# rajan-dubey8/camouflage-multimodal

Hardware: AMD Instinct MI355X
Metric: images/sec fwd+bwd (fusion model train step: fwd + loss + bwd + clip + AdamW) (higher is better)
Workload: dtype bf16; 1 GPU; BASELINE configs[1] on the path that exists (SURVEY 8d): cross-attention fusion model, packed variable-Nr minibatch (Nr ~ real 303..530 histogram, mean 483), Nk=13 real KG rows, train mode dropout 0.3, random-init weights; batch_per_gpu=16, global_batch=16, rg_dim=128, hidden_dim=256, num_heads=8, parallelism=dp1, precision=bf16 MFMA operands, fp32 accumulate/optimizer

## Files before the change

camouflage_multimodal_amd/csrc/fused_rows.h:

```cpp
#pragma once
#include "common.h"

typedef unsigned short us16;

struct ShadowJob { us16* dst; int N, K, transposed, nsrc; const float* src[4]; int rows[4]; int ld[4]; int chunk_begin; int lo; };
#define SHADOW_MAXJ 24
#define SHADOW_MAXZ 24
struct ShadowBatch { ShadowJob j[SHADOW_MAXJ]; int n; void* zero_ptr[SHADOW_MAXZ]; size_t zero_bytes[SHADOW_MAXZ]; int nzero; };
int launch_weight_shadows(ShadowBatch& sb, hipStream_t stream);

struct FrontStream {
  const float* X; int M;
  const us16* W0; const float* b0;
  const us16* W1; const float* bq; const float* bkv;
  us16* X16;
  us16* R16; us16* Q16; us16* KV16;
  int tile_begin;
};
#define FUSED_FRONT_MAXZ 4
#define FUSED_FRONT_MAXX 20
#define FUSED_BWD1_MAXZ 16
struct FrontArgs {
  FrontStream s[2]; float qscale; int save; unsigned long long* stamps; int exp;
  void* zero_ptr[FUSED_FRONT_MAXZ]; unsigned zero_bytes[FUSED_FRONT_MAXZ]; int nzero;
// ... 2 lines not shown
};
int launch_fused_front(FrontArgs& a, int variant, hipStream_t stream);

struct BackStream {
  const us16* Wo; const float* bo; const us16* W1; const float* b1; const float* ln_g; const float* ln_b;
  const us16* R16;
  us16* O16; us16* Y16; us16* XH16; float* rstd; uint32_t* mask;
  float* Ymean; float* Hmean;
  uint32_t site_ffn;
};
struct BackArgs {
  BackStream s[2];
  const us16* Q16; const us16* KV16;
  const us16* Q2_16; const us16* KV2_16;
  const int* off; const int* tile_off; const float* inv_nr;
  const int4* tile_desc;
  float* lse2;
  int lead_tiles;
  float* part; int* tickets; int max_splits;
  int B, Nk, rg_tiles_max, rows_rg;
  DropCfg drop; int save; int exp;
  unsigned long long* stamps;
  int save_lse2;
};
int launch_fused_back(BackArgs& a, int variant, int lead_mode, hipStream_t stream);

struct Bwd1Stream {
  const us16* W1T; const us16* WoT;
  const uint32_t* mask; const us16* XH16; const float* rstd; const float* ln_g;
  const float* dHm; int ld_dHm;
  const float* dcomb; int ld_dcomb;
  us16* dH16; us16* dU16;
  float* dgamma; float* dbeta;
};
struct TailWgProd { const float* dy; const float* x; float* dW; float* db; int ld_dy, ld_x, rows, cols; int tile_begin; };
#define TAIL_WG_MAXP 8
struct TailWgArgs { TailWgProd p[TAIL_WG_MAXP]; int n, B, tiles; };
struct Bwd1Args {
  Bwd1Stream s[2];
  const us16* Q16; const us16* KV16;
  us16* dQKV16; float* dKV;
  const us16* O2_16; us16* dO2_16; float* delta2;
  const int* off; const int* tile_off; const float* inv_nr; const int4* tile_desc;
  const int* row_sample;
  int B, Nk, rg_tiles_max, rows_rg; float qscale; DropCfg drop; unsigned long long* stamps;
  int exp;
// ... 44 lines not shown
```

camouflage_multimodal_amd/csrc/fused_rows.hip:

```cpp
#include "fused_rows.h"
#include "shadow_inl.h"
#include "gemm.h"
#include "mfma_inl.h"

namespace {

template <int NT, int KS, bool W_IS_A, int DEPTH, bool USE_ROT = true>
struct Stage {
  static constexpr int TOTAL = NT * KS;
  static constexpr int D = DEPTH < TOTAL ? DEPTH : TOTAL;
  static_assert(!USE_ROT || (KS & (KS - 1)) == 0, "rotated k order: power-of-two k steps");
  u32x4 buf[D];
  const u32x4* wp; int rot;
  __device__ __forceinline__ int keff(int ks) const { return USE_ROT ? ((ks + rot) & (KS - 1)) : ks; }
  __device__ __forceinline__ const u32x4* wptr(int i) const { return wp + 64 * (keff(i / NT) * NT + (i % NT)); }
  __device__ __forceinline__ void prefetch(const u32x4* __restrict__ wp_, int rot_) {
    wp = wp_; rot = rot_;
#pragma unroll
    for (int i = 0; i < D; ++i) buf[i] = *wptr(i);
  }
  __device__ __forceinline__ void run(const char* act, f32x16 (&acc)[NT]) {
    run_f([&](int ks) { return *reinterpret_cast<const bf16x8*>(act + 32 * ks); }, acc);
  }
  template <class F>
  __device__ __forceinline__ void run_f(F&& frag, f32x16 (&acc)[NT]) {
    bf16x8 x = frag(keff(0)), xn = x;
#pragma unroll
    for (int i = 0; i < TOTAL; ++i) {
      const int ks = i / NT, t = i % NT;
      const bf16x8 wf = as_frag(buf[i % D]);
      if (i + D < TOTAL) buf[i % D] = *wptr(i + D);
      if (t == 0) {
        x = xn;
        if (ks + 1 < KS) xn = frag(keff(ks + 1));
      }
      if constexpr (W_IS_A) acc[t] = __builtin_amdgcn_mfma_f32_32x32x16_bf16(wf, x, acc[t], 0, 0, 0);
      else                  acc[t] = __builtin_amdgcn_mfma_f32_32x32x16_bf16(x, wf, acc[t], 0, 0, 0);
      __builtin_amdgcn_sched_barrier(0);
    }
  }
};

__device__ __forceinline__ void stamp(unsigned long long* stamps, int k) {
  if (stamps && threadIdx.x == 0) stamps[(size_t)blockIdx.x * 8 + k] = __builtin_amdgcn_s_memrealtime();
}

template <int LOG2C>
__device__ __forceinline__ void copy_out(const char* lds, int pitch, int col_byte0, us16* dst, int ld, size_t row0, int nrows) {
  for (int c = threadIdx.x; c < (32 << LOG2C); c += 256) {
    const int r = c >> LOG2C, k = c & ((1 << LOG2C) - 1);
    if (r < nrows)
      store16_wt(reinterpret_cast<char*>(dst + (row0 + r) * (size_t)ld) + 16 * k, *reinterpret_cast<const u32x4*>(lds + r * pitch + col_byte0 + 16 * k));
  }
}
// ... 125 lines not shown
    for (int s = 0; s < 2; ++s) {
      const bf16x8 kf = *reinterpret_cast<const bf16x8*>(Ks + (l31 & 15) * PK + 2 * (32 * head + 16 * s + 8 * h));
      S = __builtin_amdgcn_mfma_f32_32x32x16_bf16(kf, qf[hd][s], S, 0, 0, 0);
    }
    float e[8];
    rg_softmax(S, h, Nk, e);
    const uint32_t ibase = ((uint32_t)(row0 + l31) * 8u + (uint32_t)head) * (uint32_t)Nk;
    if (dodrop) {
#pragma unroll
      for (int i = 0; i < 8; ++i) e[i] *= drop_mult(a.drop, SITE_ATTN_RG2KG, ibase + (uint32_t)acc_row(i, h));
    }
    const bf16x8 pf = as_frag(u32x4{pack2(e[0], e[1]), pack2(e[2], e[3]), pack2(e[4], e[5]), pack2(e[6], e[7])});
    const char* vp = Vs + (4 * h + q4) * PV + 2 * (32 * head + 16 * g1 + 4 * p4);
    const bf16x8 vf = join(lds_tr16(vp), lds_tr16(vp + 8 * PV));
    const f32x16 O = __builtin_amdgcn_mfma_f32_32x32x16_bf16(vf, pf, zero16(), 0, 0, 0);
#pragma unroll
    for (int g = 0; g < 4; ++g)
      *reinterpret_cast<u32x2*>(bufO + l31 * PR + 2 * (32 * head + 8 * g + 4 * h)) =
          u32x2{pack2(O[4 * g], O[4 * g + 1]), pack2(O[4 * g + 2], O[4 * g + 3])};
  }
}

constexpr int SPLIT_ROWS = 64;
constexpr int PART_FLOATS = 16 + 16 + 16 * 32;
static_assert(PART_FLOATS == FUSED_PART_FLOATS, "fused_rows.h");
__device__ __forceinline__ void attn_kg_split(const BackArgs& a, char* smem, int b, int sp, int w, int lane) {
  const int l31 = lane & 31, h = lane >> 5, Nk = a.Nk;
  const int rb = a.off[b], nr = a.off[b + 1] - rb, r0 = SPLIT_ROWS * sp;
  char* Vt = smem + w * (32 * PVC);
  const us16* qrow = a.Q2_16 + ((size_t)b * Nk + min(l31, Nk - 1)) * 256 + 64 * w + 8 * h;
  const us16* kbase = a.KV2_16 + (size_t)rb * 512 + 64 * w + 8 * h;
  const us16* vbase = a.KV2_16 + (size_t)rb * 512 + 256 + 64 * w;
  bf16x8 qf[2][2];
  u32x4 kf[2][2][2], vv[2][4];
#pragma unroll
  for (int hd = 0; hd < 2; ++hd)
#pragma unroll
    for (int s = 0; s < 2; ++s) qf[hd][s] = as_frag(*reinterpret_cast<const u32x4*>(qrow + 32 * hd + 16 * s));
#pragma unroll
  for (int c = 0; c < 2; ++c) {
    const us16* p = kbase + (size_t)min(r0 + 32 * c + l31, nr - 1) * 512;
#pragma unroll
    for (int hd = 0; hd < 2; ++hd)
#pragma unroll
      for (int s = 0; s < 2; ++s) kf[c][hd][s] = *reinterpret_cast<const u32x4*>(p + 32 * hd + 16 * s);
  }
// ... 50 lines not shown
  L[0] += __shfl_xor(L[0], 32, 64);
  L[1] += __shfl_xor(L[1], 32, 64);
  stamp(a.stamps, 2);
#pragma unroll
  for (int hd = 0; hd < 2; ++hd) {
    float* part = a.part + (((size_t)a.tile_off[b] + 2 * sp) * 8 + 2 * w + hd) * PART_FLOATS;
    if (lane < 16) {
      __hip_atomic_store(part + lane, mx[hd], __ATOMIC_RELAXED, __HIP_MEMORY_SCOPE_AGENT);
      __hip_atomic_store(part + 16 + lane, L[hd], __ATOMIC_RELAXED, __HIP_MEMORY_SCOPE_AGENT);
    }
    float* zt = reinterpret_cast<float*>(Vt);
#pragma unroll
    for (int i = 0; i < 8; ++i) zt[acc_row(i, h) * 32 + l31] = Z[hd][i];
#pragma unroll
    for (int r = 0; r < 2; ++r) {
      const int idx = lane + 64 * r;
      const f32x4 v = *reinterpret_cast<const f32x4*>(zt + 4 * idx);
      float* dst = part + 32 + 4 * idx;
      asm volatile("global_store_dwordx4 %0, %1, off sc1\n\ts_nop 1" ::"v"(dst), "v"(v) : "memory");
    }
  }
}

__device__ __forceinline__ void attn_kg_combine(const BackArgs& a, char* smem, char* bufO, int b, int nsplit) {
  const int tid = threadIdx.x, Nk = a.Nk;
  float* sc = reinterpret_cast<float*>(smem);
  float* invL = sc + nsplit * 128;
  const float* part = a.part + (size_t)a.tile_off[b] * 8 * PART_FLOATS;
  constexpr size_t SS = (size_t)2 * 8 * PART_FLOATS;
  f32x4 zv[4][4];
  auto load_z = [&](int s0) {
#pragma unroll
    for (int k = 0; k < 4; ++k) {
      const float* z = part + (size_t)min(s0 + k, nsplit - 1) * SS + 32;
#pragma unroll
      for (int it = 0; it < 4; ++it) {
        const int idx = tid + 256 * it;
        zv[k][it] = *reinterpret_cast<const f32x4*>(z + (size_t)(idx >> 7) * PART_FLOATS + 4 * (idx & 127));
      }
    }
  };
  load_z(0);
  if (tid < 128) {
    const int hd = tid >> 4, j = tid & 15;
    const float* p0 = part + (size_t)hd * PART_FLOATS + j;
    float M = -INFINITY, L = 0.f;
    if (nsplit <= 16) {
// ... 3 lines not shown
#pragma unroll
      for (int k = 0; k < 16; ++k) M = fmaxf(M, mv[k]);
#pragma unroll
      for (int k = 0; k < 16; ++k)
        if (k < nsplit) { const float e = __expf(mv[k] - M); sc[k * 128 + tid] = e; L = fmaf(lv[k], e, L); }
    } else {
      for (int s0 = 0; s0 < nsplit; s0 += 8) {
        float mv[8];
#pragma unroll
        for (int k = 0; k < 8; ++k) mv[k] = p0[(size_t)min(s0 + k, nsplit - 1) * SS];
#pragma unroll
        for (int k = 0; k < 8; ++k) M = fmaxf(M, mv[k]);
      }
      for (int s0 = 0; s0 < nsplit; s0 += 8) {
        float mv[8], lv[8];
#pragma unroll
        for (int k = 0; k < 8; ++k) { const size_t o = (size_t)min(s0 + k, nsplit - 1) * SS; mv[k] = p0[o]; lv[k] = p0[o + 16]; }
#pragma unroll
        for (int k = 0; k < 8; ++k)
          if (s0 + k < nsplit) { const float e = __expf(mv[k] - M); sc[(s0 + k) * 128 + tid] = e; L = fmaf(lv[k], e, L); }
      }
    }
    invL[tid] = 1.0f / L;
    if ((a.save | a.save_lse2) && a.lse2 && j < Nk) { float* o = a.lse2 + (((size_t)b * 8 + hd) * 16 + j) * 2; o[0] = M; o[1] = L; }
  }
  __syncthreads();
  f32x4 acc[4];
#pragma unroll
  for (int it = 0; it < 4; ++it) acc[it] = f32x4{0.f, 0.f, 0.f, 0.f};
  for (int s0 = 0; s0 < nsplit; s0 += 4) {
    if (s0 > 0) load_z(s0);
#pragma unroll
    for (int k = 0; k < 4; ++k)
      if (s0 + k < nsplit) {
#pragma unroll
        for (int it = 0; it < 4; ++it) acc[it] += zv[k][it] * sc[(s0 + k) * 128 + ((tid + 256 * it) >> 3)];
      }
  }
#pragma unroll
  for (int it = 0; it < 4; ++it) {
    const int idx = tid + 256 * it, hd = idx >> 7, j = (idx >> 3) & 15, f4 = idx & 7;
    if (j < Nk) {
      const float il = invL[hd * 16 + j];
      *reinterpret_cast<u32x2*>(bufO + j * PR + 2 * (32 * hd + 4 * f4)) =
          u32x2{pack2(acc[it][0] * il, acc[it][1] * il), pack2(acc[it][2] * il, acc[it][3] * il)};
    }
  }
}

template <int DEPTH, bool ROT, int OCC>
__global__ __launch_bounds__(256, OCC) void back_kernel(const BackArgs a) {
  extern __shared__ __attribute__((aligned(16))) char smem[];
  const int tid = threadIdx.x, lane = tid & 63, l31 = lane & 31, h = lane >> 5;
  const int w = __builtin_amdgcn_readfirstlane(tid >> 6);
  const int nkg = a.B * a.max_splits;
  const int vid = (int)blockIdx.x < a.lead_tiles ? nkg + (int)blockIdx.x : ((int)blockIdx.x < a.lead_tiles + nkg ? (int)blockIdx.x - a.lead_tiles : (int)blockIdx.x);
  const bool kg = vid < nkg;
  int rot = ROT ? (int)(blockIdx.x >> 3) : 0;
  using L = BackL<OCC>;
  char* bufO = smem + L::O; char* bufY = smem + L::Y;
  float* red = reinterpret_cast<float*>(smem + L::RED);
  float* tile32 = reinterpret_cast<float*>(smem);
  int b; size_t rowg0; int nrows; float inv_n;
  stamp(a.stamps, 0);
  const BackStream& S = a.s[kg ? 1 : 0];
  Stage<2, 16, true, DEPTH> sto;
  Stage<4, 16, false, DEPTH> stf;
  if (!kg) sto.prefetch(reinterpret_cast<const u32x4*>(S.Wo) + (size_t)w * (16 * 2 * 64) + lane, rot);
  if (kg) {
    b = vid / a.max_splits;
    const int sp = vid - b * a.max_splits;
    if (ROT) rot = b;
    const int nsplit = (a.off[b + 1] - a.off[b] + SPLIT_ROWS - 1) / SPLIT_ROWS;
    if (sp >= nsplit) return;
    attn_kg_split(a, smem, b, sp, w, lane);
    stamp(a.stamps, 4);
    asm volatile("s_waitcnt vmcnt(0)" ::: "memory");
    __syncthreads();
    int* flag = reinterpret_cast<int*>(red);
    if (tid == 0) flag[0] = __hip_atomic_fetch_add(a.tickets + b, 1, __ATOMIC_RELAXED, __HIP_MEMORY_SCOPE_AGENT);
    __syncthreads();
    stamp(a.stamps, 5);
    if (flag[0] != nsplit - 1) return;
    if (tid == 0) {
      __builtin_amdgcn_fence(__ATOMIC_ACQUIRE, "agent");
      asm volatile("s_waitcnt vmcnt(0)" ::: "memory");
    }
    for (int c = tid; c < 32 * PR / 16; c += 256) reinterpret_cast<u32x4*>(bufO)[c] = u32x4{0u, 0u, 0u, 0u};
    __syncthreads();
    sto.prefetch(reinterpret_cast<const u32x4*>(S.Wo) + (size_t)w * (16 * 2 * 64) + lane, rot);
    attn_kg_combine(a, smem, bufO, b, nsplit);
    stamp(a.stamps, 6);
    rowg0 = (size_t)b * a.Nk; nrows = a.Nk; inv_n = 1.0f / (float)a.Nk;
  } else {
    const int4 td = a.tile_desc[vid - nkg];
    if (td.x < 0) return;
    b = td.x; rowg0 = td.y; nrows = td.z; inv_n = __int_as_float(td.w);
    attn_rg_tile(a, smem, bufO, b, rowg0, nrows, w, lane);
  }
  __syncthreads();
  stamp(a.stamps, 1);

  const size_t rrow = rowg0 + min(l31, nrows - 1);
  float u[32];
  float rstd_keep = 0.f;
  {
    f32x16 acc[2] = {zero16(), zero16()};
    sto.run(bufO + l31 * PR + 16 * h, acc);
    stf.prefetch(reinterpret_cast<const u32x4*>(S.W1) + (size_t)w * (16 * 4 * 64) + lane, rot);
    float part = 0.f;
#pragma unroll
    for (int t = 0; t < 2; ++t)
#pragma unroll
      for (int g = 0; g < 4; ++g) {
        const int c0 = 64 * w + 32 * t + 8 * g + 4 * h;
        const float4 bv = *reinterpret_cast<const float4*>(S.bo + c0);
        const u32x2 rv = *reinterpret_cast<const u32x2*>(S.R16 + rrow * 256 + c0);
        float* o = u + 16 * t + 4 * g;
        o[0] = acc[t][4 * g] + bv.x + bf_lo(rv.x); o[1] = acc[t][4 * g + 1] + bv.y + bf_hi(rv.x);
        o[2] = acc[t][4 * g + 2] + bv.z + bf_lo(rv.y); o[3] = acc[t][4 * g + 3] + bv.w + bf_hi(rv.y);
        part += (o[0] + o[1]) + (o[2] + o[3]);
      }
    auto row_total = [&](float p, int slot) {
      p += __shfl_xor(p, 32, 64);
      if (h == 0) red[slot * 128 + w * 32 + l31] = p;
      __syncthreads();
      return (red[slot * 128 + l31] + red[slot * 128 + 32 + l31]) + (red[slot * 128 + 64 + l31] + red[slot * 128 + 96 + l31]);
    };
    const float mean = row_total(part, 0) * (1.0f / 256.0f);
    float sq = 0.f;
#pragma unroll
    for (int i = 0; i < 32; ++i) { u[i] -= mean; sq = fmaf(u[i], u[i], sq); }
// ... 12 lines not shown
        const float4 y = make_float4(x0 * gm.x + bt.x, x1 * gm.y + bt.y, x2 * gm.z + bt.z, x3 * gm.w + bt.w);
        *reinterpret_cast<u32x2*>(bufY + l31 * PR + 2 * c0) = u32x2{pack2(y.x, y.y), pack2(y.z, y.w)};
        if constexpr (OCC == 3) {
          ys[4 * g] = rok ? y.x : 0.f; ys[4 * g + 1] = rok ? y.y : 0.f; ys[4 * g + 2] = rok ? y.z : 0.f; ys[4 * g + 3] = rok ? y.w : 0.f;
          if (a.save) *reinterpret_cast<u32x2*>(smem + L::XH + l31 * PR + 2 * c0) = u32x2{pack2(x0, x1), pack2(x2, x3)};
        } else {
          *reinterpret_cast<float4*>(tile32 + l31 * PT + c0) = y;
          o[0] = x0; o[1] = x1; o[2] = x2; o[3] = x3;
        }
      }
      if constexpr (OCC == 2) continue;
#pragma unroll
      for (int st = 0; st < 4; ++st) {
        const int n = 8 >> st, m = 16 >> st;
        const bool up = (l31 & m) != 0;
#pragma unroll
        for (int i = 0; i < n; ++i) {
          const float send = up ? ys[i] : ys[i + n];
          const float keep = up ? ys[i + n] : ys[i];
          ys[i] = keep + __shfl_xor(send, m, 64);
        }
      }
      const float tot = ys[0] + __shfl_xor(ys[0], 1, 64);
      if ((l31 & 1) == 0) {
        const int i16 = (l31 >> 1) & 15;
        atomicAdd(S.Ymean + (size_t)b * 256 + 64 * w + 32 * t + 8 * (i16 >> 2) + 4 * h + (i16 & 3), tot * inv_n);
      }
    }
  }
  __syncthreads();
  stamp(a.stamps, 2);
  if constexpr (OCC == 2) {
    float sum = 0.f;
    for (int r = 0; r < nrows; ++r) sum += tile32[r * PT + tid];
    atomicAdd(S.Ymean + (size_t)b * 256 + tid, sum * inv_n);
  }

  {
    f32x16 acc[4] = {zero16(), zero16(), zero16(), zero16()};
    stf.run(bufY + l31 * PR + 16 * h, acc);
    const bool dodrop = a.drop.p > 0.f;
#pragma unroll
    for (int t = 0; t < 4; ++t) {
      const int f = 128 * w + 32 * t + l31;
      const float bias = S.b1[f];
      float colsum = 0.f;
      uint32_t wlo = 0u, whi = 0u;
#pragma unroll
      for (int i = 0; i < 16; ++i) {
        if (8 * (i >> 2) >= nrows) continue;
        const int row = acc_row(i, h);
        float v = fmaxf(acc[t][i] + bias, 0.f);
        if (dodrop) v *= drop_mult(a.drop, S.site_ffn, (uint32_t)(rowg0 + row) * 512u + (uint32_t)f);
        if (row >= nrows) v = 0.f;
        colsum += v;
        if (a.save) {
          const unsigned long long bal = __ballot(v > 0.f);
          SET_LANE(wlo, (uint32_t)bal, i); SET_LANE(whi, (uint32_t)(bal >> 32), i);
        }
      }
      colsum += __shfl_xor(colsum, 32, 64);
      if (h == 0) atomicAdd(S.Hmean + (size_t)b * 512 + f, colsum * inv_n);
      if (a.save && lane < 16) {
        const int ra = acc_row(lane, 0);
        if (ra < nrows) S.mask[(rowg0 + ra) * 16 + 4 * w + t] = wlo;
        if (ra + 4 < nrows) S.mask[(rowg0 + ra + 4) * 16 + 4 * w + t] = whi;
      }
    }
  }
  if (a.save) {
    char* bufXH = smem + L::XH;
    if (w == 0 && h == 0 && l31 < nrows) S.rstd[rowg0 + l31] = rstd_keep;
    __syncthreads();
    if constexpr (OCC == 2) {
#pragma unroll
      for (int t = 0; t < 2; ++t)
#pragma unroll
        for (int g = 0; g < 4; ++g) {
          const float* o = u + 16 * t + 4 * g;
          *reinterpret_cast<u32x2*>(bufXH + l31 * PR + 2 * (64 * w + 32 * t + 8 * g + 4 * h)) = u32x2{pack2(o[0], o[1]), pack2(o[2], o[3])};
        }
      __syncthreads();
    }
    copy_out<5>(bufXH, PR, 0, S.XH16, 256, rowg0, nrows);
    copy_out<5>(bufO, PR, 0, S.O16, 256, rowg0, nrows);
    copy_out<5>(bufY, PR, 0, S.Y16, 256, rowg0, nrows);
  }
  stamp(a.stamps, 3);
}


constexpr int W_GTAB = 0, W_BUFDU = 1024, W_KS = W_BUFDU + 32 * PR, W_VS = W_KS + 16 * PK, W_BUFDO = W_VS + 16 * PK,
              W_IMGS = W_BUFDO + 32 * PR, W_RED = W_IMGS + 16384, W_LDS = W_RED + 1024;
// ... 763 lines not shown
    total += (S.M + 31) / 32;
  }
  if (a.nzero < 0 || a.nzero > FUSED_FRONT_MAXZ) return (int)hipErrorInvalidValue;
  for (int i = 0; i < a.nzero; ++i)
    if (!a.zero_ptr[i] || !al16(a.zero_ptr[i]) || (a.zero_bytes[i] & 15)) return (int)hipErrorInvalidValue;
  const int prof = gemm_prof_open(stream, 2.0 * ((double)a.s[0].M + a.s[1].M) * (128.0 * 256.0 + 256.0 * 768.0), PROF_FRONT);
  if (variant == 0)      launch_lds<front_kernel<12, false>>(dim3(total), dim3(256), F_LDS, stream, a);
  else if (variant != 2) launch_lds<front_kernel<12, true>>(dim3(total), dim3(256), F_LDS, stream, a);
  else                   launch_lds<front_kernel<16, true>>(dim3(total), dim3(256), F_LDS, stream, a);
  gemm_prof_close(prof, stream);
  return (int)hipGetLastError();
}

int launch_fused_back(BackArgs& a, int variant, int lead_mode, hipStream_t stream) {
  if (a.B < 1 || a.Nk < 1 || a.Nk > 16 || a.rg_tiles_max < 1 || !a.Q16 || !a.KV16 || !a.Q2_16 || !a.KV2_16 || !a.off || !a.tile_off || !a.tile_desc || !a.inv_nr ||
      !a.part || !a.tickets || a.max_splits < 1 || a.max_splits > FUSED_MAX_SPLITS)
    return (int)hipErrorInvalidValue;
  for (int i = 0; i < 2; ++i) {
    const BackStream& S = a.s[i];
    if (!S.Wo || !S.bo || !S.W1 || !S.b1 || !S.ln_g || !S.ln_b || !S.R16 || !S.Ymean || !S.Hmean) return (int)hipErrorInvalidValue;
    if (a.save && (!S.O16 || !S.Y16 || !S.XH16 || !S.rstd || !S.mask)) return (int)hipErrorInvalidValue;
    if (!al16(S.bo) || !al16(S.ln_g) || !al16(S.ln_b) || !al16(S.Wo) || !al16(S.W1) || !al16(S.R16)) return (int)hipErrorInvalidValue;
  }
  const dim3 grid(a.B * a.max_splits + a.rg_tiles_max);
  a.lead_tiles = (lead_mode != 0 && a.rows_rg / 32 >= 256 && (int)grid.x > 512) ? 256 : 0;
  const double rows = (double)a.rows_rg + (double)a.B * a.Nk;
  const int prof = gemm_prof_open(stream, 2.0 * rows * (256.0 * 256.0 + 256.0 * 512.0) + 8.0 * (double)a.rows_rg * a.Nk * 256.0, PROF_BACK);
  if (variant == 0)        launch_lds<back_kernel<12, false, 2>>(grid, dim3(256), BackL<2>::LDS, stream, a);
  else if (variant != 2) {
    if (grid.x <= 512u)    launch_lds<back_kernel<12, true, 2>>(grid, dim3(256), BackL<2>::LDS, stream, a);
    else                   launch_lds<back_kernel<12, true, 3>>(grid, dim3(256), BackL<3>::LDS, stream, a);
  } else                   launch_lds<back_kernel<16, true, 2>>(grid, dim3(256), BackL<2>::LDS, stream, a);
  gemm_prof_close(prof, stream);
  return (int)hipGetLastError();
}

size_t fused_bwd1_lds() { return W_LDS; }

int launch_fused_bwd1(Bwd1Args& a, int variant, hipStream_t stream, int kg_only) {
  if (a.B < 1 || a.Nk < 1 || a.Nk > 16 || a.rg_tiles_max < 1 || !a.Q16 || !a.KV16 || !a.dQKV16 || !a.dKV || !a.O2_16 || !a.dO2_16 || !a.delta2 ||
      !a.off || !a.tile_off || !a.tile_desc || !a.inv_nr || !a.row_sample)
    return (int)hipErrorInvalidValue;
  for (int i = 0; i < 2; ++i) {
    const Bwd1Stream& S = a.s[i];
    if (!S.W1T || !S.WoT || !S.mask || !S.XH16 || !S.rstd || !S.ln_g || !S.dHm || !S.dcomb || !S.dH16 || !S.dU16 || !S.dgamma || !S.dbeta)
      return (int)hipErrorInvalidValue;
    if (!al16(S.W1T) || !al16(S.WoT) || !al16(S.mask) || !al16(S.ln_g) || !al16(S.dcomb) || (S.ld_dcomb & 3) || !al16(S.dH16) || !al16(S.dU16))
      return (int)hipErrorInvalidValue;
// ... 48 lines not shown
```

camouflage_multimodal_amd/csrc/fusion_abi.hip:

```cpp
#include <hip/hip_runtime.h>

#include <algorithm>
#include <cmath>
#include <cstdio>
#include <cstring>
#include <string>

#include "../../include/camo_fusion.h"

#include "attn.h"
#include "gemm.h"
#include "fused_rows.h"
#include "tail_wide.h"
#include "attn_maps.h"
#include "gemm16.h"
#include "misc.h"
#include "abi_util.h"
#include "fusion_ws.h"

namespace {
thread_local std::string g_err;
}

int camo_abi::fail(int code, const std::string& msg) { g_err = msg; return code; }
// ... 419 lines not shown
      xj(tp.Wfu0[lo], H, 2 * H, 0, P[CAMO_P_FU_W0], lo); xj(tp.Wfu3[lo], H, H, 0, P[CAMO_P_FU_W3], lo);
    }
    for (int lo = 0; lo < 2; ++lo) xheads(tp.Wh0[lo], 2 * H, H, 0, lo);
    if (pl.tail != CAMO_TAIL_PLANES)
      for (int lo = 0; lo < 2; ++lo) {
        xheads(tp.Wh0T[lo], H, 2 * H, 1, lo);
        xj(tp.Wfu3T[lo], H, H, 1, P[CAMO_P_FU_W3], lo);
        xj(tp.Wfu0T[lo], 2 * H, H, 1, P[CAMO_P_FU_W0], lo);
        xj(tp.W13T[lo], 2 * H, H, 1, P[CAMO_P_F1_W3], lo);
        xj(tp.W23T[lo], 2 * H, H, 1, P[CAMO_P_F2_W3], lo);
      }
  }
  if (pl.front == CAMO_FRONT_KG) { fa.split3 = 1; CK(launch_wide_front(fa, 1, st, 1), "fused forward, KG rows' front half (32-row tiles, one in-projection pass per block)"); }
  else if (pl.front == CAMO_FRONT_WIDE) CK(launch_wide_front(fa, pl.front_rt, st, 0), "fused forward, front half (wide tiles)");
  else CK(launch_fused_front(fa, x.opt->fused_variant, st), "fused forward, front half");
  BackArgs ba; std::memset(&ba, 0, sizeof(ba));
  ba.s[0] = BackStream{sh.Wo1, P[CAMO_P_A1_OUT_B], sh.W1, P[CAMO_P_F1_B0], P[CAMO_P_LN1_W], P[CAMO_P_LN1_B], f.R16,
                       f.O16, f.Y16, f.XH16, f.rstd1, f.mask1, w.Ymean, w.H1mean, SITE_FFN_RG};
  ba.s[1] = BackStream{sh.Wo2, P[CAMO_P_A2_OUT_B], sh.W2, P[CAMO_P_F2_B0], P[CAMO_P_LN2_W], P[CAMO_P_LN2_B], f.G16,
                       f.O2_16, f.Y2_16, f.XH2_16, f.rstd2, f.mask2, w.Y2mean, w.H2mean, SITE_FFN_KG};
  ba.Q16 = f.Q16; ba.KV16 = f.KV16; ba.Q2_16 = f.Q2_16; ba.KV2_16 = f.KV2_16;
  ba.off = x.rg_offsets; ba.tile_off = x.bd.tile_off; ba.tile_desc = x.bd.tile_desc; ba.inv_nr = x.bd.inv_nr; ba.lse2 = f.lse2;
  ba.B = B; ba.Nk = Nk; ba.rows_rg = T; ba.rg_tiles_max = T / 32 + B;
  ba.part = f.part; ba.tickets = w.tickets; ba.max_splits = (max_nr + 63) / 64;
  ba.drop = x.drop; ba.save = save ? 1 : 0; ba.save_lse2 = pl.maps; ba.exp = x.opt->exp;
  ba.stamps = g_dbg_stamps ? g_dbg_stamps + (size_t)g_dbg_stamp_blocks * 8 : nullptr;
  switch (pl.back) {
    case CAMO_BACK_RG_64: CK(launch_wide2_rgfwd(fa.s[0], sh.Wf_rg, sh.bf_rg, fa.qscale, ba, max_nr, pl.save_r16, st), "fused forward, RG rows in one launch (64-row half-blocks)"); break;
    case CAMO_BACK_RG_WIDE: CK(launch_wide_rgfwd(fa.s[0], fa.qscale, ba, pl.back_rt, max_nr, st), "fused forward, RG rows in one launch (wide tiles)"); break;
    case CAMO_BACK_WIDE: CK(launch_wide_back(ba, pl.back_rt, max_nr, st), "fused forward, back half (wide tiles)"); break;
    default: CK(launch_fused_back(ba, x.opt->fused_variant, x.opt->back_lead, st), "fused forward, back half");
  }
  if (pl.maps) {
    AttnMapsArgs ma; std::memset(&ma, 0, sizeof(ma));
    ma.Q16 = f.Q16; ma.KV16 = f.KV16; ma.Q2_16 = f.Q2_16; ma.KV2_16 = f.KV2_16; ma.lse2 = f.lse2; ma.tile_desc = x.bd.tile_desc;
    ma.rg2kg = attn_rg2kg; ma.kg2rg = attn_kg2rg; ma.Nk = Nk; ma.tiles = T / 32 + B; ma.rows_rg = T;
    CK(launch_attn_maps(ma, st), "attention maps of the fused forward");
  }
  return 0;
}

int record_tail_event(const Call& c, hipStream_t st) { return c.tail_event ? (int)hipEventRecord(c.tail_event, st) : 0; }

int backward_nodes16(const Batch& x) {
  const camo_dims_t& d = *x.dims; const float* const* P = x.P; float* const* Gr = x.Gr; const Ws& w = x.w; const DropCfg& drop = x.drop; hipStream_t st = x.st;
  const int32_t* rg_offsets = x.rg_offsets; const int32_t* row_sample = x.bd.row_sample; const float* inv_nr = x.bd.inv_nr;
  const int B = x.B, T = x.T, Nk = x.Nk;
// ... 698 lines not shown
```

camouflage_multimodal_amd/csrc/fusion_ws.h:

```cpp
#pragma once
#include <cstring>

#include "../../include/camo_fusion.h"
#include "abi_util.h"
#include "fused_rows.h"

namespace camo_ws {
using camo_abi::Carver;

struct Take : Carver {
  using Carver::Carver;
  template <typename T> void operator()(T*& p, size_t n, const char* = nullptr) { p = take<T>(n); }
  void name(const void*, const char*) {}
};
struct Find : Carver {
  const char* want; const void* hit = nullptr;
  Find(void* base, const char* w) : Carver(base), want(w) {}
  template <typename T> void operator()(T*& p, size_t n, const char* nm = nullptr) { p = take<T>(n); name(p, nm); }
  void name(const void* p, const char* nm) { if (nm && std::strcmp(nm, want) == 0) hit = p; }
};
template <class C> struct Members {
  C& c; float* base; size_t words = 0;
  template <typename T> void operator()(T*& p, size_t n, const char* nm = nullptr) { p = base ? reinterpret_cast<T*>(base + words) : nullptr; words += n; c.name(p, nm); }
  size_t bytes() const { return words * sizeof(float); }
// ... 54 lines not shown
constexpr bool shadow_slices_ordered() {
  for (int i = 0, at = 0; i < 10; at += k_shadow_slices[i++].rows) {
    const ShadowSlice& s = k_shadow_slices[i];
    if (i && s.plain != k_shadow_slices[i - 1].plain) at = 0;
    if (s.pn0 != at || (s.trans && s.tk0 != at)) return false;
  }
  return true;
}
static_assert(shadow_slices_ordered(), "slices of one shadow must be adjacent and ascend in n0 = k0");

inline size_t tail_counter_words(int B) { return (size_t)4 * ((B + 15) / 16 > 0 ? (B + 15) / 16 : 1); }

struct Range { void* ptr; size_t bytes; };
struct PadRows { Range r[18]; int n; };
struct HiLo {
  us16 *hi, *lo;
  us16* operator[](int low) const { return low ? lo : hi; }
};

struct Ws {
  float* zero_base; size_t zero_bytes, zero_fwd_bytes;
  float *Ymean, *H1mean, *Y2mean, *H2mean, *dfused, *dKV;
  int* tickets;
  float* dQ2acc;
  struct TailSum { float *F1sum, *hidsum, *dF1sum; unsigned int* counters; size_t bytes; } tailsum;
  struct ParM { float *Mrg, *Mkg, *dbrg, *dbkg; } parM;
  float *R, *G, *Q, *KV2, *KV, *Q2, *P, *P2, *O, *O2, *U, *U2, *st1, *st2, *Y, *Y2, *H1, *H2;
  float *comb, *F1, *fused, *hid, *a2;
  float *dlog, *dhid, *dF1, *dcomb, *dHm1, *dHm2, *da2;
  float *dH1, *dH2, *dY, *dY2, *dU, *dU2, *dO, *dO2, *dQ, *dQ2, *dKV2, *dS2, *dR, *dG;
  struct H16 {
    us16 *X, *KG, *R, *G, *O, *O2, *Y, *Y2, *dH1, *dH2, *dU, *dU2, *dQKV, *dQKVkg, *dR, *dG;
    us16 *H1, *H2;
    us16 *Wrg, *Wkg, *Win1, *Win2, *Wo1, *Wo2, *W1, *W2, *W1T, *W2T, *Wo1T, *Wo2T, *WcRgT, *WcKgT;
    PadRows pad;
  } h;
  struct F17 {
    ShadowSet sh;
    us16 *X16, *KG16, *R16, *G16, *Q16, *Q2_16, *KV16, *KV2_16, *O16, *O2_16, *Y16, *Y2_16, *XH16, *XH2_16;
    float *rstd1, *rstd2, *lse2, *part; uint32_t *mask1, *mask2;
    us16 *dH16, *dH2_16, *dU16, *dU2_16, *dQKV16, *dQKVkg16, *dR16, *dG16, *dO2_16;
    float *delta2, *dGpart;
    PadRows pad;
    struct TailPlanes { HiLo W13, W23, Wfu0, Wfu3, Wh0, Wh0T, Wfu3T, Wfu0T, W13T, W23T; } tp;
  } f;
  size_t bytes;
};

enum { RG_ROWS = 0, KG_ROWS = 1 };

template <class C> Ws carve_with(C& c, const camo_dims_t& d, int B, int T, int Nk) {
  Ws w{};
  const size_t H = d.hidden_dim, TK = (size_t)B * Nk, nh = d.num_heads, Wd = 2 * d.num_classes + 2;
  if (d.fusion_type == CAMO_FUSION_CROSS_ATTENTION) {
    const size_t Fh = H / 2;
    c(w.R, T * H, "R"); c(w.G, TK * H, "G"); c(w.Q, T * H, "Q"); c(w.KV2, T * 2 * H, "KV2"); c(w.KV, TK * 2 * H, "KV"); c(w.Q2, TK * H, "Q2");
    c(w.P, T * nh * Nk, "P"); c(w.P2, T * nh * Nk, "P2"); c(w.O, T * H, "O"); c(w.O2, TK * H, "O2"); c(w.U, T * H, "U"); c(w.U2, TK * H, "U2");
    c(w.st1, T * 2); c(w.st2, TK * 2); c(w.Y, T * H, "Y"); c(w.Y2, TK * H, "Y2"); c(w.H1, T * 2 * H, "H1"); c(w.H2, TK * 2 * H, "H2");
    {
      c(w.zero_base, 0);
      Members<C> z{c, w.zero_base};
      z(w.Ymean, B * H, "Ymean"); z(w.H1mean, B * 2 * H, "H1mean"); z(w.Y2mean, B * H, "Y2mean"); z(w.H2mean, B * 2 * H, "H2mean");
      z(w.dfused, B * H, "dfused");
      z(w.tickets, ((size_t)2 * B + 3) & ~size_t(3));
      w.zero_fwd_bytes = z.bytes();
      z(w.dKV, TK * 2 * H, "dKV"); z(w.dQ2acc, TK * H, "dQ2acc");
      Ws::TailSum& t = w.tailsum;
      const size_t t0 = z.bytes();
      z(t.F1sum, B * H); z(t.hidsum, B * 2 * H); z(t.dF1sum, B * H); z(t.counters, (tail_counter_words(B) + 3) & ~size_t(3));
      t.bytes = z.bytes() - t0;
      const size_t D = d.rg_dim;
      z(w.parM.Mrg, 3 * H * D); z(w.parM.Mkg, 3 * H * D); z(w.parM.dbrg, 3 * H); z(w.parM.dbkg, 3 * H + 8);
      w.zero_bytes = z.bytes(); c.off += w.zero_bytes;
    }
    c(w.comb, B * 2 * H, "comb"); c(w.F1, B * H, "F1"); c(w.fused, B * H, "fused"); c(w.hid, B * 4 * Fh, "hid");
    c(w.dlog, B * Wd); c(w.dhid, B * 4 * Fh, "dhid"); c(w.dF1, B * H, "dF1"); c(w.dcomb, B * 2 * H, "dcomb");
    c(w.dHm1, B * 2 * H, "dHm1"); c(w.dHm2, B * 2 * H, "dHm2");
    c(w.dH1, T * 2 * H); c(w.dH2, TK * 2 * H); c(w.dY, T * H); c(w.dY2, TK * H); c(w.dU, T * H); c(w.dU2, TK * H); c(w.dO, T * H); c(w.dO2, TK * H);
    c(w.dQ, T * H); c(w.dQ2, TK * H); c(w.dKV2, T * 2 * H); c(w.dS2, T * nh * Nk); c(w.dR, T * H); c(w.dG, TK * H);
    const size_t Tp = ((size_t)T + 127) / 128 * 128, TKp = (TK + 127) / 128 * 128, D = d.rg_dim, Dk = d.kg_dim;
    auto rows16 = [&](us16*& p, int stream, size_t width, PadRows* pads, const char* nm = nullptr) {
      const size_t rows = stream == KG_ROWS ? TK : (size_t)T, rows_p = stream == KG_ROWS ? TKp : Tp;
      c(p, rows_p * width, nm);
      if (pads) pads->r[pads->n++] = Range{p ? p + rows * width : nullptr, (rows_p - rows) * width * sizeof(us16)};
    };
    Ws::H16& h = w.h;
    rows16(h.X, RG_ROWS, D, &h.pad); rows16(h.KG, KG_ROWS, Dk, &h.pad); rows16(h.R, RG_ROWS, H, &h.pad); rows16(h.G, KG_ROWS, H, &h.pad);
// ... 54 lines not shown
```

Measured before the change: 97460 images/s.

## Split KG-row FFN tail across helper blocks that claim column slices

Adds per-sample helper blocks to the fused back kernel. After the last KG split finishes the combine, it closes a claim counter and publishes how many helpers joined. Each helper redoes the combine and Wo projection, then computes only its slice of the 512-wide FFN (W1) columns, so the serial critical-path tail per sample is shortened. The cost is spin-waiting on atomics, redundant combine/Wo work per helper, extra grid blocks and a new zeroed claim buffer. Helpers that time out poison Hmean with NaN.

```diff
diff --git a/camouflage_multimodal_amd/csrc/fused_rows.h b/camouflage_multimodal_amd/csrc/fused_rows.h
--- a/camouflage_multimodal_amd/csrc/fused_rows.h
+++ b/camouflage_multimodal_amd/csrc/fused_rows.h
@@ -48,6 +48,8 @@
   DropCfg drop; int save; int exp;
   unsigned long long* stamps;
   int save_lse2;
+  int* claim;
+  int helpers;
 };
 int launch_fused_back(BackArgs& a, int variant, int lead_mode, hipStream_t stream);
 
diff --git a/camouflage_multimodal_amd/csrc/fused_rows.hip b/camouflage_multimodal_amd/csrc/fused_rows.hip
--- a/camouflage_multimodal_amd/csrc/fused_rows.hip
+++ b/camouflage_multimodal_amd/csrc/fused_rows.hip
@@ -7,29 +7,33 @@
 
 template <int NT, int KS, bool W_IS_A, int DEPTH, bool USE_ROT = true>
 struct Stage {
-  static constexpr int TOTAL = NT * KS;
-  static constexpr int D = DEPTH < TOTAL ? DEPTH : TOTAL;
+  static constexpr int D = DEPTH < NT * KS ? DEPTH : NT * KS;
   static_assert(!USE_ROT || (KS & (KS - 1)) == 0, "rotated k order: power-of-two k steps");
   u32x4 buf[D];
   const u32x4* wp; int rot;
   __device__ __forceinline__ int keff(int ks) const { return USE_ROT ? ((ks + rot) & (KS - 1)) : ks; }
-  __device__ __forceinline__ const u32x4* wptr(int i) const { return wp + 64 * (keff(i / NT) * NT + (i % NT)); }
+  template <int NR>
+  __device__ __forceinline__ const u32x4* wptr(int i) const { return wp + 64 * (keff(i / NR) * NT + (i % NR)); }
+  template <int NR = NT>
   __device__ __forceinline__ void prefetch(const u32x4* __restrict__ wp_, int rot_) {
+    static_assert(NR >= 1 && NR <= NT && D <= NR * KS, "a narrower run keeps the stage's buffer depth");
     wp = wp_; rot = rot_;
 #pragma unroll
-    for (int i = 0; i < D; ++i) buf[i] = *wptr(i);
-  }
-  __device__ __forceinline__ void run(const char* act, f32x16 (&acc)[NT]) {
-    run_f([&](int ks) { return *reinterpret_cast<const bf16x8*>(act + 32 * ks); }, acc);
-  }
-  template <class F>
-  __device__ __forceinline__ void run_f(F&& frag, f32x16 (&acc)[NT]) {
+    for (int i = 0; i < D; ++i) buf[i] = *wptr<NR>(i);
+  }
+  template <int NR = NT>
+  __device__ __forceinline__ void run(const char* act, f32x16 (&acc)[NR]) {
+    run_f<NR>([&](int ks) { return *reinterpret_cast<const bf16x8*>(act + 32 * ks); }, acc);
+  }
+  template <int NR = NT, class F>
+  __device__ __forceinline__ void run_f(F&& frag, f32x16 (&acc)[NR]) {
+    constexpr int TOTAL = NR * KS;
     bf16x8 x = frag(keff(0)), xn = x;
 #pragma unroll
     for (int i = 0; i < TOTAL; ++i) {
-      const int ks = i / NT, t = i % NT;
+      const int ks = i / NR, t = i % NR;
       const bf16x8 wf = as_frag(buf[i % D]);
-      if (i + D < TOTAL) buf[i % D] = *wptr(i + D);
+      if (i + D < TOTAL) buf[i % D] = *wptr<NR>(i + D);
       if (t == 0) {
         x = xn;
         if (ks + 1 < KS) xn = frag(keff(ks + 1));
@@ -201,6 +205,10 @@
 }
 
 constexpr int SPLIT_ROWS = 64;
+constexpr int KGH_CLOSED = 1 << 16, KGH_SPINS = 1 << 16;
+constexpr int KGH_DEFAULT_P = 2;
+constexpr int KGH_EXP_P1 = 0x100, KGH_EXP_P2 = 0x200, KGH_EXP_P4 = 0x400, KGH_EXP_LATE = 0x800;
+template <int N> struct IntC { static constexpr int value = N; };
 constexpr int PART_FLOATS = 16 + 16 + 16 * 32;
 static_assert(PART_FLOATS == FUSED_PART_FLOATS, "fused_rows.h");
 __device__ __forceinline__ void attn_kg_split(const BackArgs& a, char* smem, int b, int sp, int w, int lane) {
@@ -297,7 +305,7 @@
   }
 }
 
-__device__ __forceinline__ void attn_kg_combine(const BackArgs& a, char* smem, char* bufO, int b, int nsplit) {
+__device__ __forceinline__ void attn_kg_combine(const BackArgs& a, char* smem, char* bufO, int b, int nsplit, bool write_lse2) {
   const int tid = threadIdx.x, Nk = a.Nk;
   float* sc = reinterpret_cast<float*>(smem);
   float* invL = sc + nsplit * 128;
@@ -347,7 +355,7 @@
       }
     }
     invL[tid] = 1.0f / L;
-    if ((a.save | a.save_lse2) && a.lse2 && j < Nk) { float* o = a.lse2 + (((size_t)b * 8 + hd) * 16 + j) * 2; o[0] = M; o[1] = L; }
+    if (write_lse2 && (a.save | a.save_lse2) && a.lse2 && j < Nk) { float* o = a.lse2 + (((size_t)b * 8 + hd) * 16 + j) * 2; o[0] = M; o[1] = L; }
   }
   __syncthreads();
   f32x4 acc[4];
@@ -379,8 +387,9 @@
   const int tid = threadIdx.x, lane = tid & 63, l31 = lane & 31, h = lane >> 5;
   const int w = __builtin_amdgcn_readfirstlane(tid >> 6);
   const int nkg = a.B * a.max_splits;
+  const bool helper = (int)blockIdx.x >= nkg + a.rg_tiles_max;
   const int vid = (int)blockIdx.x < a.lead_tiles ? nkg + (int)blockIdx.x : ((int)blockIdx.x < a.lead_tiles + nkg ? (int)blockIdx.x - a.lead_tiles : (int)blockIdx.x);
-  const bool kg = vid < nkg;
+  const bool kg = helper || vid < nkg;
   int rot = ROT ? (int)(blockIdx.x >> 3) : 0;
   using L = BackL<OCC>;
   char* bufO = smem + L::O; char* bufY = smem + L::Y;
@@ -392,29 +401,66 @@
   Stage<2, 16, true, DEPTH> sto;
   Stage<4, 16, false, DEPTH> stf;
   if (!kg) sto.prefetch(reinterpret_cast<const u32x4*>(S.Wo) + (size_t)w * (16 * 2 * 64) + lane, rot);
+  int npart = 1, part = 0;
   if (kg) {
-    b = vid / a.max_splits;
-    const int sp = vid - b * a.max_splits;
-    if (ROT) rot = b;
-    const int nsplit = (a.off[b + 1] - a.off[b] + SPLIT_ROWS - 1) / SPLIT_ROWS;
-    if (sp >= nsplit) return;
-    attn_kg_split(a, smem, b, sp, w, lane);
-    stamp(a.stamps, 4);
-    asm volatile("s_waitcnt vmcnt(0)" ::: "memory");
-    __syncthreads();
     int* flag = reinterpret_cast<int*>(red);
-    if (tid == 0) flag[0] = __hip_atomic_fetch_add(a.tickets + b, 1, __ATOMIC_RELAXED, __HIP_MEMORY_SCOPE_AGENT);
-    __syncthreads();
-    stamp(a.stamps, 5);
-    if (flag[0] != nsplit - 1) return;
+    int nsplit;
+    if (!helper) {
+      b = vid / a.max_splits;
+      const int sp = vid - b * a.max_splits;
+      if (ROT) rot = b;
+      nsplit = (a.off[b + 1] - a.off[b] + SPLIT_ROWS - 1) / SPLIT_ROWS;
+      if (sp >= nsplit) return;
+      attn_kg_split(a, smem, b, sp, w, lane);
+      stamp(a.stamps, 4);
+      asm volatile("s_waitcnt vmcnt(0)" ::: "memory");
+      __syncthreads();
+      if (tid == 0) flag[0] = __hip_atomic_fetch_add(a.tickets + b, 1, __ATOMIC_RELAXED, __HIP_MEMORY_SCOPE_AGENT);
+      __syncthreads();
+      stamp(a.stamps, 5);
+      if (flag[0] != nsplit - 1) return;
+    } else {
+      b = ((int)blockIdx.x - nkg - a.rg_tiles_max) % a.B;
+      if (ROT) rot = b;
+      nsplit = (a.off[b + 1] - a.off[b] + SPLIT_ROWS - 1) / SPLIT_ROWS;
+      if (tid == 0) {
+        int P = 0;
+        const int r = a.exp == KGH_EXP_LATE ? KGH_CLOSED : __hip_atomic_fetch_add(a.claim + b, 1, __ATOMIC_RELAXED, __HIP_MEMORY_SCOPE_AGENT);
+        if (!(r & KGH_CLOSED)) {
+          stamp(a.stamps, 5);
+          for (int spins = 0; (P = __hip_atomic_load(a.claim + a.B + b, __ATOMIC_RELAXED, __HIP_MEMORY_SCOPE_AGENT)) == 0;) {
+            __builtin_amdgcn_s_sleep(2);
+            if (++spins > KGH_SPINS) { P = -1; break; }
+          }
+          if (r >= a.helpers || P > a.helpers + 1) P = -1;
+        }
+        flag[0] = P; flag[2] = r + 1;
+      }
+      __syncthreads();
+      if (flag[0] == 0) { stamp(a.stamps, 7); return; }
+      if (flag[0] < 0) {
+        for (int f = tid; f < 512; f += 256) atomicAdd(a.s[1].Hmean + (size_t)b * 512 + f, __int_as_float(0x7fc00000));
+        return;
+      }
+      stamp(a.stamps, 4);
+    }
     if (tid == 0) {
+      if (!helper) {
+        int n = 0;
+        if (a.helpers) {
+          n = __hip_atomic_fetch_or(a.claim + b, KGH_CLOSED, __ATOMIC_RELAXED, __HIP_MEMORY_SCOPE_AGENT) & (KGH_CLOSED - 1);
+          if (n) __hip_atomic_store(a.claim + a.B + b, 1 + n, __ATOMIC_RELAXED, __HIP_MEMORY_SCOPE_AGENT);
+        }
+        flag[1] = 1 + n; flag[2] = 0;
+      } else flag[1] = flag[0];
       __builtin_amdgcn_fence(__ATOMIC_ACQUIRE, "agent");
       asm volatile("s_waitcnt vmcnt(0)" ::: "memory");
     }
     for (int c = tid; c < 32 * PR / 16; c += 256) reinterpret_cast<u32x4*>(bufO)[c] = u32x4{0u, 0u, 0u, 0u};
     __syncthreads();
+    npart = __builtin_amdgcn_readfirstlane(flag[1]); part = __builtin_amdgcn_readfirstlane(flag[2]);
     sto.prefetch(reinterpret_cast<const u32x4*>(S.Wo) + (size_t)w * (16 * 2 * 64) + lane, rot);
-    attn_kg_combine(a, smem, bufO, b, nsplit);
+    attn_kg_combine(a, smem, bufO, b, nsplit, !helper);
     stamp(a.stamps, 6);
     rowg0 = (size_t)b * a.Nk; nrows = a.Nk; inv_n = 1.0f / (float)a.Nk;
   } else {
@@ -429,10 +475,16 @@
   const size_t rrow = rowg0 + min(l31, nrows - 1);
   float u[32];
   float rstd_keep = 0.f;
+  int ntw, g0;
   {
     f32x16 acc[2] = {zero16(), zero16()};
     sto.run(bufO + l31 * PR + 16 * h, acc);
-    stf.prefetch(reinterpret_cast<const u32x4*>(S.W1) + (size_t)w * (16 * 4 * 64) + lane, rot);
+    ntw = npart == 1 ? 4 : ((npart == 2 || (npart == 3 && part == 0)) ? 2 : 1);
+    g0 = (npart == 3 ? (part == 0 ? 0 : 4 + 4 * part) : 4 * ntw * part) + ntw * w;
+    const u32x4* wp1 = reinterpret_cast<const u32x4*>(S.W1) + (size_t)(g0 >> 2) * (16 * 4 * 64) + 64 * (g0 & 3) + lane;
+    if (ntw == 4) stf.prefetch(wp1, rot);
+    else if (ntw == 2) stf.template prefetch<2>(wp1, rot);
+    else stf.template prefetch<1>(wp1, rot);
     float part = 0.f;
 #pragma unroll
     for (int t = 0; t < 2; ++t)
@@ -491,7 +543,7 @@
         }
       }
       const float tot = ys[0] + __shfl_xor(ys[0], 1, 64);
-      if ((l31 & 1) == 0) {
+      if ((l31 & 1) == 0 && !helper) {
         const int i16 = (l31 >> 1) & 15;
         atomicAdd(S.Ymean + (size_t)b * 256 + 64 * w + 32 * t + 8 * (i16 >> 2) + 4 * h + (i16 & 3), tot * inv_n);
       }
@@ -499,19 +551,20 @@
   }
   __syncthreads();
   stamp(a.stamps, 2);
-  if constexpr (OCC == 2) {
+  if (OCC == 2 && !helper) {
     float sum = 0.f;
     for (int r = 0; r < nrows; ++r) sum += tile32[r * PT + tid];
     atomicAdd(S.Ymean + (size_t)b * 256 + tid, sum * inv_n);
   }
 
   {
-    f32x16 acc[4] = {zero16(), zero16(), zero16(), zero16()};
-    stf.run(bufY + l31 * PR + 16 * h, acc);
-    const bool dodrop = a.drop.p > 0.f;
-#pragma unroll
-    for (int t = 0; t < 4; ++t) {
-      const int f = 128 * w + 32 * t + l31;
+    DropCfg drop = a.drop;
+    uint32_t site = S.site_ffn;
+    int save = a.save;
+    asm volatile("" : "+s"(drop.seed_lo), "+s"(drop.seed_hi), "+s"(drop.thr), "+s"(drop.scale), "+s"(site), "+s"(save));
+    const bool dodrop = drop.p > 0.f;
+    auto epilogue = [&](const f32x16& acc, int g) __attribute__((always_inline)) {
+      const int f = 32 * g + l31;
       const float bias = S.b1[f];
       float colsum = 0.f;
       uint32_t wlo = 0u, whi = 0u;
@@ -519,25 +572,37 @@
       for (int i = 0; i < 16; ++i) {
         if (8 * (i >> 2) >= nrows) continue;
         const int row = acc_row(i, h);
-        float v = fmaxf(acc[t][i] + bias, 0.f);
-        if (dodrop) v *= drop_mult(a.drop, S.site_ffn, (uint32_t)(rowg0 + row) * 512u + (uint32_t)f);
+        float v = fmaxf(acc[i] + bias, 0.f);
+        if (dodrop) v *= drop_mult(drop, site, (uint32_t)(rowg0 + row) * 512u + (uint32_t)f);
         if (row >= nrows) v = 0.f;
         colsum += v;
-        if (a.save) {
+        if (save) {
           const unsigned long long bal = __ballot(v > 0.f);
           SET_LANE(wlo, (uint32_t)bal, i); SET_LANE(whi, (uint32_t)(bal >> 32), i);
         }
       }
       colsum += __shfl_xor(colsum, 32, 64);
       if (h == 0) atomicAdd(S.Hmean + (size_t)b * 512 + f, colsum * inv_n);
-      if (a.save && lane < 16) {
+      if (save && lane < 16) {
         const int ra = acc_row(lane, 0);
-        if (ra < nrows) S.mask[(rowg0 + ra) * 16 + 4 * w + t] = wlo;
-        if (ra + 4 < nrows) S.mask[(rowg0 + ra + 4) * 16 + 4 * w + t] = whi;
-      }
-    }
-  }
-  if (a.save) {
+        if (ra < nrows) S.mask[(rowg0 + ra) * 16 + g] = wlo;
+        if (ra + 4 < nrows) S.mask[(rowg0 + ra + 4) * 16 + g] = whi;
+      }
+    };
+    auto layer = [&](auto nr) __attribute__((always_inline)) {
+      constexpr int NR = decltype(nr)::value;
+      f32x16 acc[NR];
+#pragma unroll
+      for (int t = 0; t < NR; ++t) acc[t] = zero16();
+      stf.template run<NR>(bufY + l31 * PR + 16 * h, acc);
+#pragma unroll
+      for (int t = 0; t < NR; ++t) epilogue(acc[t], g0 + t);
+    };
+    if (ntw == 4) layer(IntC<4>{});
+    else if (ntw == 2) layer(IntC<2>{});
+    else layer(IntC<1>{});
+  }
+  if (a.save && !helper) {
     char* bufXH = smem + L::XH;
     if (w == 0 && h == 0 && l31 < nrows) S.rstd[rowg0 + l31] = rstd_keep;
     __syncthreads();
@@ -1347,8 +1412,11 @@
     if (a.save && (!S.O16 || !S.Y16 || !S.XH16 || !S.rstd || !S.mask)) return (int)hipErrorInvalidValue;
     if (!al16(S.bo) || !al16(S.ln_g) || !al16(S.ln_b) || !al16(S.Wo) || !al16(S.W1) || !al16(S.R16)) return (int)hipErrorInvalidValue;
   }
-  const dim3 grid(a.B * a.max_splits + a.rg_tiles_max);
+  dim3 grid(a.B * a.max_splits + a.rg_tiles_max);
   a.lead_tiles = (lead_mode != 0 && a.rows_rg / 32 >= 256 && (int)grid.x > 512) ? 256 : 0;
+  const int P = a.exp == KGH_EXP_P1 ? 1 : (a.exp == KGH_EXP_P2 ? 2 : (a.exp == KGH_EXP_P4 ? 4 : KGH_DEFAULT_P));
+  a.helpers = (a.claim && P > 1 && a.lead_tiles == 0 && (int)grid.x + a.B * (P - 1) <= 512) ? P - 1 : 0;
+  grid.x += a.B * a.helpers;
   const double rows = (double)a.rows_rg + (double)a.B * a.Nk;
   const int prof = gemm_prof_open(stream, 2.0 * rows * (256.0 * 256.0 + 256.0 * 512.0) + 8.0 * (double)a.rows_rg * a.Nk * 256.0, PROF_BACK);
   if (variant == 0)        launch_lds<back_kernel<12, false, 2>>(grid, dim3(256), BackL<2>::LDS, stream, a);
diff --git a/camouflage_multimodal_amd/csrc/fusion_abi.hip b/camouflage_multimodal_amd/csrc/fusion_abi.hip
--- a/camouflage_multimodal_amd/csrc/fusion_abi.hip
+++ b/camouflage_multimodal_amd/csrc/fusion_abi.hip
@@ -465,7 +465,7 @@
   ba.Q16 = f.Q16; ba.KV16 = f.KV16; ba.Q2_16 = f.Q2_16; ba.KV2_16 = f.KV2_16;
   ba.off = x.rg_offsets; ba.tile_off = x.bd.tile_off; ba.tile_desc = x.bd.tile_desc; ba.inv_nr = x.bd.inv_nr; ba.lse2 = f.lse2;
   ba.B = B; ba.Nk = Nk; ba.rows_rg = T; ba.rg_tiles_max = T / 32 + B;
-  ba.part = f.part; ba.tickets = w.tickets; ba.max_splits = (max_nr + 63) / 64;
+  ba.part = f.part; ba.tickets = w.tickets; ba.claim = w.kg_claim; ba.max_splits = (max_nr + 63) / 64;
   ba.drop = x.drop; ba.save = save ? 1 : 0; ba.save_lse2 = pl.maps; ba.exp = x.opt->exp;
   ba.stamps = g_dbg_stamps ? g_dbg_stamps + (size_t)g_dbg_stamp_blocks * 8 : nullptr;
   switch (pl.back) {
diff --git a/camouflage_multimodal_amd/csrc/fusion_ws.h b/camouflage_multimodal_amd/csrc/fusion_ws.h
--- a/camouflage_multimodal_amd/csrc/fusion_ws.h
+++ b/camouflage_multimodal_amd/csrc/fusion_ws.h
@@ -100,6 +100,7 @@
   float* zero_base; size_t zero_bytes, zero_fwd_bytes;
   float *Ymean, *H1mean, *Y2mean, *H2mean, *dfused, *dKV;
   int* tickets;
+  int* kg_claim;
   float* dQ2acc;
   struct TailSum { float *F1sum, *hidsum, *dF1sum; unsigned int* counters; size_t bytes; } tailsum;
   struct ParM { float *Mrg, *Mkg, *dbrg, *dbkg; } parM;
@@ -141,6 +142,7 @@
       z(w.Ymean, B * H, "Ymean"); z(w.H1mean, B * 2 * H, "H1mean"); z(w.Y2mean, B * H, "Y2mean"); z(w.H2mean, B * 2 * H, "H2mean");
       z(w.dfused, B * H, "dfused");
       z(w.tickets, ((size_t)2 * B + 3) & ~size_t(3));
+      z(w.kg_claim, ((size_t)2 * B + 3) & ~size_t(3), "kg_claim");
       w.zero_fwd_bytes = z.bytes();
       z(w.dKV, TK * 2 * H, "dKV"); z(w.dQ2acc, TK * H, "dQ2acc");
       Ws::TailSum& t = w.tailsum;
```

Result: no change. 97840 images/s (median of 5 runs) (+0.4%).
